# itshawi/data-accelerator

Measured on AMD Instinct MI355X. Metric: events/sec (node) + p99 latency, SimulatedData IoT Flow, higher is better.
Workload: dtype fp64/int64 columns (no reduced precision)

## Files before the change

dxa/ops/csrc/inflate.hip:

```cpp
#include "dxa_common.h"

namespace {

constexpr int IG = 16;
constexpr int WG = 128;
constexpr int LBITS = 9;
constexpr int DBITS = 8;
constexpr int kWaitVm0 = 0xF70;

enum : int32_t { IF_OK = 0, IF_TRUNC = 1, IF_DIST = 2, IF_OVERFLOW = 3, IF_SIZE = 4, IF_CODE = 10, IF_BLOCK = 6 };

struct Tables {
  uint16_t lfast[1 << LBITS];
  uint16_t dfast[1 << DBITS];
  uint16_t lsorted[288];
  uint16_t dsorted[32];
  uint16_t lcount[16];
  uint16_t dcount[16];
  uint8_t lens[320];
  uint8_t clens[20];
  uint16_t csorted[19];
  uint16_t ccount[16];
};

__constant__ uint16_t kLenBase[29] = {3,  4,  5,  6,  7,  8,  9,  10, 11,  13,  15,  17,  19,  23, 27,
                                      31, 35, 43, 51, 59, 67, 83, 99, 115, 131, 163, 195, 227, 258};
__constant__ uint8_t kLenExtra[29] = {0, 0, 0, 0, 0, 0, 0, 0, 1, 1, 1, 1, 2, 2, 2, 2, 3, 3, 3, 3, 4, 4, 4, 4, 5, 5, 5, 5, 0};
__constant__ uint16_t kDistBase[30] = {1,   2,   3,   4,   5,   7,    9,    13,   17,   25,   33,   49,    65,    97,    129,
                                       193, 257, 385, 513, 769, 1025, 1537, 2049, 3073, 4097, 6145, 8193, 12289, 16385, 24577};
__constant__ uint8_t kDistExtra[30] = {0, 0, 0, 0, 1, 1, 2, 2, 3, 3, 4, 4, 5, 5, 6, 6, 7, 7, 8, 8, 9, 9, 10, 10, 11, 11, 12, 12, 13, 13};
__constant__ uint8_t kClenOrder[19] = {16, 17, 18, 0, 8, 7, 9, 6, 10, 5, 11, 4, 12, 3, 13, 2, 14, 1, 15};

__device__ __forceinline__ uint32_t bitrev(uint32_t c, int n) { return __builtin_bitreverse32(c) >> (32 - n); }

__device__ __forceinline__ void lane_sync() {
  __builtin_amdgcn_fence(__ATOMIC_RELEASE, "wavefront");
  __builtin_amdgcn_wave_barrier();
  __builtin_amdgcn_fence(__ATOMIC_ACQUIRE, "wavefront");
}

__device__ bool build_table(const uint8_t* lens, int n, uint16_t* count, uint16_t* sorted, uint16_t* fast, int bits,
                            int maxlen, int gl) {
  lane_sync();
  if (fast) {
    for (int i = gl; i < (1 << bits); i += IG) fast[i] = 0;
    lane_sync();
  }
  uint16_t cnt[16];
  for (int l = 0; l < 16; ++l) cnt[l] = 0;
  for (int s = 0; s < n; ++s) cnt[lens[s]]++;
  int left = 1;
  for (int l = 1; l <= maxlen; ++l) {
    left = (left << 1) - cnt[l];
    if (left < 0) return false;
  }
  uint16_t offs[16];
  offs[1] = 0;
  for (int l = 1; l < 15; ++l) offs[l + 1] = offs[l] + cnt[l];
  if (gl == 0) {
    for (int l = 0; l < 16; ++l) count[l] = cnt[l];
  }
  uint32_t next[16];
  uint32_t code = 0;
  next[0] = 0;
  for (int l = 1; l < 16; ++l) {
    next[l] = code;
    code = (code + cnt[l]) << 1;
  }
  for (int s = 0; s < n; ++s) {
    const int l = lens[s];
    if (!l) continue;
    if (gl == 0) sorted[offs[l]] = (uint16_t)s;
    offs[l]++;
    const uint32_t c = next[l]++;
    if (fast && l <= bits) {
      const uint32_t r = bitrev(c, l);
      const uint16_t e = (uint16_t)((l << 9) | s);
      for (int k = gl; k < (1 << (bits - l)); k += IG) fast[r | ((uint32_t)k << l)] = e;
    }
  }
  lane_sync();
  return true;
}

__global__ __launch_bounds__(WG) void inflate_group_kernel(const uint8_t* __restrict__ src,
                                                           const int64_t* __restrict__ comp_off,
                                                           const int32_t* __restrict__ comp_len,
                                                           const uint8_t* __restrict__ kind,
                                                           const int64_t* __restrict__ out_off,
                                                           const int64_t* __restrict__ cap_arr, int64_t nb,
                                                           uint8_t* __restrict__ dst, int64_t* __restrict__ produced,
                                                           int32_t* __restrict__ status) {
  __shared__ Tables tabs[WG / IG];
  Tables& T = tabs[threadIdx.x / IG];
  const int64_t b = ((int64_t)blockIdx.x * WG + threadIdx.x) / IG;
  const int gl = (int)(threadIdx.x & (IG - 1));
  if (b >= nb || kind[b] != 2) return;
  const uint8_t* in = src + comp_off[b];
  const int32_t n = comp_len[b];
  const int64_t cap64 = cap_arr[b];
  uint8_t* out = dst + out_off[b];
  if (n < 0 || cap64 < 0 || cap64 > INT32_MAX) {
    if (gl == 0) status[b] = IF_OVERFLOW;
    return;
  }
  const int32_t cap = (int32_t)cap64;
  const int32_t lim = n + 8;
  uint64_t bb = 0;
  int bc = 0;
  int32_t ip = 0;
  auto ld32 = [&](int32_t p) -> uint32_t {
    if (p + 4 <= lim) {
      const uintptr_t a = reinterpret_cast<uintptr_t>(in + p);
      const uint32_t* w = reinterpret_cast<const uint32_t*>(a & ~(uintptr_t)3);
      const uint32_t sh = (uint32_t)(a & 3) * 8u;
      const uint32_t lo = w[0];
      if (!sh) return lo;
      return (lo >> sh) | (w[1] << (32u - sh));
    }
    uint32_t v = 0;
    for (int i = 0; i < 4; ++i)
      if (p + i < lim) v |= (uint32_t)in[p + i] << (8 * i);
    return v;
  };
  auto refill = [&]() {
    if (bc <= 32) {
      bb |= (uint64_t)ld32(ip) << bc;
      ip += 4;
      bc += 32;
    }
  };
  auto bits = [&](int k) -> uint32_t {
    refill();
    const uint32_t v = (uint32_t)(bb & ((1ull << k) - 1));
    bb >>= k;
    bc -= k;
    return v;
  };
  auto slow = [&](const uint16_t* count, const uint16_t* sorted, int maxlen) -> int {
    refill();
    int code = 0, first = 0, index = 0;
    for (int l = 1; l <= maxlen; ++l) {
      code |= (int)(bb & 1);
      bb >>= 1;
      bc--;
      const int c = count[l];
      if (code - first < c) return sorted[index + code - first];
      index += c;
      first = (first + c) << 1;
      code <<= 1;
    }
    return -1;
  };
  auto decode = [&](const uint16_t* fast, int fbits, const uint16_t* count, const uint16_t* sorted) -> int {
    refill();
    const uint32_t e = fast[bb & ((1u << fbits) - 1)];
    const int l = (int)(e >> 9);
    if (l) {
      bb >>= l;
      bc -= l;
      return (int)(e & 511);
    }
    return slow(count, sorted, 15);
  };
  int32_t op = 0, rc = IF_OK, done = 0;
  bool last = false;
  while (!last && rc == IF_OK) {
    if ((int64_t)ip * 8 - bc > (int64_t)lim * 8) { rc = IF_TRUNC; break; }
    last = bits(1) != 0;
    const uint32_t type = bits(2);
    if (type == 0) {
      const int drop = bc & 7;
      bb >>= drop;
      bc -= drop;
      const uint32_t len = bits(16), nlen = bits(16);
      if ((len ^ 0xffffu) != nlen) { rc = IF_BLOCK; break; }
      const int32_t pos = ip - bc / 8;
      if (pos + (int32_t)len > n) { rc = IF_TRUNC; break; }
      if (op + (int32_t)len > cap) { rc = IF_OVERFLOW; break; }
      for (int32_t c = gl; c < (int32_t)len; c += IG) out[op + c] = in[pos + c];
      op += (int32_t)len;
      ip = pos + (int32_t)len;
      bb = 0;
      bc = 0;
      continue;
    }
    if (type == 3) { rc = IF_BLOCK; break; }
    int nlit = 288, ndist = 30;
    if (type == 1) {
      for (int s = gl; s < 320; s += IG) T.lens[s] = s < 144 ? 8 : s < 256 ? 9 : s < 280 ? 7 : s < 288 ? 8 : 5;
    } else {
      nlit = (int)bits(5) + 257;
      ndist = (int)bits(5) + 1;
      const int ncl = (int)bits(4) + 4;
      if (nlit > 286 || ndist > 30) { rc = IF_BLOCK; break; }
      uint32_t cl[19];
      for (int i = 0; i < 19; ++i) cl[i] = 0;
      for (int i = 0; i < ncl; ++i) cl[kClenOrder[i]] = bits(3);
      if (gl == 0) {
        for (int i = 0; i < 19; ++i) T.clens[i] = (uint8_t)cl[i];
      }
      if (!build_table(T.clens, 19, T.ccount, T.csorted, nullptr, 0, 7, gl)) { rc = IF_CODE + 0; break; }
      int i = 0;
      while (i < nlit + ndist) {
        const int sym = slow(T.ccount, T.csorted, 7);
        if (sym < 0) { rc = IF_CODE + 1; break; }
        if (sym < 16) {
          if (gl == 0) T.lens[i] = (uint8_t)sym;
          ++i;
          continue;
        }
        int rep, val = 0;
        if (sym == 16) {
          if (i == 0) { rc = IF_CODE + 2; break; }
          lane_sync();
          val = T.lens[i - 1];
          rep = 3 + (int)bits(2);
        } else if (sym == 17) {
          rep = 3 + (int)bits(3);
        } else {
          rep = 11 + (int)bits(7);
        }
        if (i + rep > nlit + ndist) { rc = IF_CODE + 3; break; }
        for (int k = gl; k < rep; k += IG) T.lens[i + k] = (uint8_t)val;
        i += rep;
      }
      if (rc != IF_OK) break;
      lane_sync();
      if (T.lens[256] == 0) { rc = IF_CODE + 4; break; }
    }
    if (!build_table(T.lens, nlit, T.lcount, T.lsorted, T.lfast, LBITS, 15, gl) ||
        !build_table(T.lens + nlit, ndist, T.dcount, T.dsorted, T.dfast, DBITS, 15, gl)) {
      rc = IF_CODE + 5;
      break;
    }
    for (;;) {
      if ((int64_t)ip * 8 - bc > (int64_t)lim * 8) { rc = IF_TRUNC; break; }
      const int sym = decode(T.lfast, LBITS, T.lcount, T.lsorted);
      if (sym < 0) { rc = IF_CODE + 6; break; }
      if (sym < 256) {
        if (op >= cap) { rc = IF_OVERFLOW; break; }
        if (gl == 0) out[op] = (uint8_t)sym;
        ++op;
        continue;
      }
      if (sym == 256) break;
      const int li = sym - 257;
      if (li >= 29) { rc = IF_CODE + 7; break; }
      const int32_t len = kLenBase[li] + (int32_t)bits(kLenExtra[li]);
      const int ds = decode(T.dfast, DBITS, T.dcount, T.dsorted);
      if (ds < 0 || ds >= 30) { rc = IF_CODE + 8; break; }
      const int32_t dist = kDistBase[ds] + (int32_t)bits(kDistExtra[ds]);
      if (dist > op) { rc = IF_DIST; break; }
      if (len > cap - op) { rc = IF_OVERFLOW; break; }
      const int32_t s0 = op - dist;
      if (s0 + (dist < len ? dist : len) > done) {
        __builtin_amdgcn_s_waitcnt(kWaitVm0);
        asm volatile("" ::: "memory");
        done = op;
      }
      if (dist >= len) {
        for (int32_t c = 0; c < len; c += IG)
          if (c + gl < len) out[op + c + gl] = out[s0 + c + gl];
      } else {
        for (int32_t c = 0; c < len; c += IG) {
          const uint32_t k = (uint32_t)(c + gl);
          if ((int32_t)k < len) out[op + (int32_t)k] = out[s0 + (int32_t)(k % (uint32_t)dist)];
        }
      }
      op += len;
    }
  }
  if (rc == IF_OK && op != cap) rc = IF_SIZE;
  if (gl == 0) {
    status[b] = rc;
    produced[b] = op;
  }
}

}

DXA_API int dxa_inflate_into(const void* src, const void* comp_off, const void* comp_len, const void* kind,
                             const void* out_off, const void* cap, int64_t nb, void* dst, void* produced, void* status,
                             void* st) {
  if (nb <= 0) return 0;
  hipLaunchKernelGGL(inflate_group_kernel, dim3((unsigned)((nb * IG + WG - 1) / WG)), dim3(WG), 0, (hipStream_t)st,
                     (const uint8_t*)src, (const int64_t*)comp_off, (const int32_t*)comp_len, (const uint8_t*)kind,
                     (const int64_t*)out_off, (const int64_t*)cap, nb, (uint8_t*)dst, (int64_t*)produced,
                     (int32_t*)status);
  return (int)hipGetLastError();
}
```

Baseline: 251.8 million.

## Stage compressed input via cooperative lane windows and parallelize Huffman table build

Replaces per-lane unaligned 32-bit input loads with a cooperative scheme: each of the 16 lanes in a group loads one word of a 16-word window, and the bit reader pulls words through ds_bpermute, prefetching the next window. Huffman table construction is parallelized with shared atomic histograms and per-length sorted fill, and fast-table entries now pre-encode length and distance base and extra-bit info so the constant-memory lookups go away. Match copies defer their store by one iteration so the load and store overlap. This adds complexity and cross-lane shuffles, and the bit-reader edge cases and delayed-store ordering bring correctness risk.

```diff
diff --git a/dxa/ops/csrc/inflate.hip b/dxa/ops/csrc/inflate.hip
--- a/dxa/ops/csrc/inflate.hip
+++ b/dxa/ops/csrc/inflate.hip
@@ -21,15 +21,39 @@
   uint8_t clens[20];
   uint16_t csorted[19];
   uint16_t ccount[16];
+  uint32_t bcnt[16];
+  uint16_t boffs[16];
+  uint16_t bnext[16];
 };
 
-__constant__ uint16_t kLenBase[29] = {3,  4,  5,  6,  7,  8,  9,  10, 11,  13,  15,  17,  19,  23, 27,
-                                      31, 35, 43, 51, 59, 67, 83, 99, 115, 131, 163, 195, 227, 258};
-__constant__ uint8_t kLenExtra[29] = {0, 0, 0, 0, 0, 0, 0, 0, 1, 1, 1, 1, 2, 2, 2, 2, 3, 3, 3, 3, 4, 4, 4, 4, 5, 5, 5, 5, 0};
-__constant__ uint16_t kDistBase[30] = {1,   2,   3,   4,   5,   7,    9,    13,   17,   25,   33,   49,    65,    97,    129,
-                                       193, 257, 385, 513, 769, 1025, 1537, 2049, 3073, 4097, 6145, 8193, 12289, 16385, 24577};
-__constant__ uint8_t kDistExtra[30] = {0, 0, 0, 0, 1, 1, 2, 2, 3, 3, 4, 4, 5, 5, 6, 6, 7, 7, 8, 8, 9, 9, 10, 10, 11, 11, 12, 12, 13, 13};
-__constant__ uint8_t kClenOrder[19] = {16, 17, 18, 0, 8, 7, 9, 6, 10, 5, 11, 4, 12, 3, 13, 2, 14, 1, 15};
+enum : int { K_PLAIN = 0, K_LITLEN = 1, K_DIST = 2 };
+constexpr uint32_t E_SPECIAL = 0x8000u;
+
+constexpr uint64_t kClenOrderLo = 16ull | 17ull << 5 | 18ull << 10 | 0ull << 15 | 8ull << 20 | 7ull << 25 | 9ull << 30 |
+                                  6ull << 35 | 10ull << 40 | 5ull << 45 | 11ull << 50 | 4ull << 55;
+constexpr uint64_t kClenOrderHi = 12ull | 3ull << 5 | 13ull << 10 | 2ull << 15 | 14ull << 20 | 1ull << 25 | 15ull << 30;
+
+__device__ __forceinline__ int clen_order(int i) {
+  return (int)((i < 12 ? kClenOrderLo >> (5 * i) : kClenOrderHi >> (5 * (i - 12))) & 31);
+}
+
+__device__ __forceinline__ uint32_t lentry(int s) {
+  if (s < 256) return (uint32_t)s << 4;
+  if (s == 256) return E_SPECIAL | (7u << 12);
+  const int li = s - 257;
+  if (li >= 29) return E_SPECIAL | (6u << 12);
+  if (li == 28) return E_SPECIAL | (255u << 4);
+  const int x = li < 4 ? 0 : (li >> 2) - 1;
+  const int base3 = li < 4 ? li : (4 + (li & 3)) << x;
+  return E_SPECIAL | ((uint32_t)x << 12) | ((uint32_t)base3 << 4);
+}
+
+__device__ __forceinline__ uint32_t dentry(int s) {
+  if (s >= 30) return E_SPECIAL;
+  const int x = s < 2 ? 0 : (s >> 1) - 1;
+  const int m = s < 2 ? s : 2 | (s & 1);
+  return ((uint32_t)m << 8) | ((uint32_t)x << 4);
+}
 
 __device__ __forceinline__ uint32_t bitrev(uint32_t c, int n) { return __builtin_bitreverse32(c) >> (32 - n); }
 
@@ -39,44 +63,53 @@
   __builtin_amdgcn_fence(__ATOMIC_ACQUIRE, "wavefront");
 }
 
-__device__ bool build_table(const uint8_t* lens, int n, uint16_t* count, uint16_t* sorted, uint16_t* fast, int bits,
-                            int maxlen, int gl) {
+template <int KIND>
+__device__ bool build_table(Tables& T, const uint8_t* lens, int n, uint16_t* count, uint16_t* sorted, uint16_t* fast,
+                            int bits, int maxlen, int gl) {
+  T.bcnt[gl] = 0;
+  if (fast) {
+    for (int i = gl; i < (1 << bits); i += IG) fast[i] = 0;
+  }
+  lane_sync();
+  for (int s = gl; s < n; s += IG) atomicAdd(&T.bcnt[lens[s] & 15], 1u);
+  lane_sync();
+  int left = 1;
+  bool ok = true;
+  uint32_t off = 0, code = 0, slot = 0;
+  for (int l = 1; l < 16; ++l) {
+    const uint32_t c = T.bcnt[l];
+    if (l <= maxlen) {
+      left = (left << 1) - (int)c;
+      ok = ok && left >= 0;
+    }
+    if (gl == l) {
+      slot = off;
+      T.boffs[l] = (uint16_t)off;
+      T.bnext[l] = (uint16_t)code;
+      count[l] = (uint16_t)c;
+    }
+    off += c;
+    code = (code + c) << 1;
+  }
+  if (!ok) return false;
+  if (gl == 0) {
+    count[0] = (uint16_t)T.bcnt[0];
+  } else {
+#pragma unroll 4
+    for (int s = 0; s < n; ++s) {
+      if (lens[s] == gl) sorted[slot++] = (uint16_t)s;
+    }
+  }
   lane_sync();
   if (fast) {
-    for (int i = gl; i < (1 << bits); i += IG) fast[i] = 0;
-    lane_sync();
-  }
-  uint16_t cnt[16];
-  for (int l = 0; l < 16; ++l) cnt[l] = 0;
-  for (int s = 0; s < n; ++s) cnt[lens[s]]++;
-  int left = 1;
-  for (int l = 1; l <= maxlen; ++l) {
-    left = (left << 1) - cnt[l];
-    if (left < 0) return false;
-  }
-  uint16_t offs[16];
-  offs[1] = 0;
-  for (int l = 1; l < 15; ++l) offs[l + 1] = offs[l] + cnt[l];
-  if (gl == 0) {
-    for (int l = 0; l < 16; ++l) count[l] = cnt[l];
-  }
-  uint32_t next[16];
-  uint32_t code = 0;
-  next[0] = 0;
-  for (int l = 1; l < 16; ++l) {
-    next[l] = code;
-    code = (code + cnt[l]) << 1;
-  }
-  for (int s = 0; s < n; ++s) {
-    const int l = lens[s];
-    if (!l) continue;
-    if (gl == 0) sorted[offs[l]] = (uint16_t)s;
-    offs[l]++;
-    const uint32_t c = next[l]++;
-    if (fast && l <= bits) {
+    for (uint32_t j = gl; j < off; j += IG) {
+      const int s = sorted[j];
+      const int l = lens[s] & 15;
+      if (l > bits) continue;
+      const uint32_t c = (uint32_t)T.bnext[l] + (j - T.boffs[l]);
       const uint32_t r = bitrev(c, l);
-      const uint16_t e = (uint16_t)((l << 9) | s);
-      for (int k = gl; k < (1 << (bits - l)); k += IG) fast[r | ((uint32_t)k << l)] = e;
+      const uint16_t e = (uint16_t)((KIND == K_LITLEN ? lentry(s) : dentry(s)) | (uint32_t)l);
+      for (uint32_t k = 0; k < (1u << (bits - l)); ++k) fast[r | (k << l)] = e;
     }
   }
   lane_sync();
@@ -100,45 +133,68 @@
   const int32_t n = comp_len[b];
   const int64_t cap64 = cap_arr[b];
   uint8_t* out = dst + out_off[b];
-  if (n < 0 || cap64 < 0 || cap64 > INT32_MAX) {
+  if (n < 0 || n > INT32_MAX - 64 || cap64 < 0 || cap64 > INT32_MAX) {
     if (gl == 0) status[b] = IF_OVERFLOW;
     return;
   }
   const int32_t cap = (int32_t)cap64;
   const int32_t lim = n + 8;
+  const int32_t skip = (int32_t)(reinterpret_cast<uintptr_t>(in) & 3);
+  const uint32_t* w = reinterpret_cast<const uint32_t*>(in - skip);
+  const int32_t avail = skip + lim;
+  const int32_t nfull = avail >> 2;
+  uint32_t tail = 0;
+  for (int i = 0; i < (avail & 3); ++i) tail |= (uint32_t)in[nfull * 4 - skip + i] << (8 * i);
+  auto ldw = [&](int32_t k) -> uint32_t { return w[k < nfull ? k : nfull - 1]; };
+  const int lbase = (int)(threadIdx.x & 63 & ~(IG - 1)) << 2;
   uint64_t bb = 0;
   int bc = 0;
-  int32_t ip = 0;
-  auto ld32 = [&](int32_t p) -> uint32_t {
-    if (p + 4 <= lim) {
-      const uintptr_t a = reinterpret_cast<uintptr_t>(in + p);
-      const uint32_t* w = reinterpret_cast<const uint32_t*>(a & ~(uintptr_t)3);
-      const uint32_t sh = (uint32_t)(a & 3) * 8u;
-      const uint32_t lo = w[0];
-      if (!sh) return lo;
-      return (lo >> sh) | (w[1] << (32u - sh));
-    }
-    uint32_t v = 0;
-    for (int i = 0; i < 4; ++i)
-      if (p + i < lim) v |= (uint32_t)in[p + i] << (8 * i);
-    return v;
+  int32_t wn = 0;
+  uint32_t cur = 0, nwin = 0, nxt = 0;
+  auto raw = [&](int32_t k) -> uint32_t {
+    return (uint32_t)__builtin_amdgcn_ds_bpermute(lbase + ((k & (IG - 1)) << 2), (int)cur);
+  };
+  auto pick = [&](uint32_t v, int32_t k) -> uint32_t {
+    return k < nfull ? v : k == nfull ? tail : 0u;
+  };
+  auto fetch = [&]() {
+    if ((wn & (IG - 1)) == 0) {
+      asm volatile("v_mov_b32 %0, %1" : "=v"(cur) : "v"(nwin));
+      nwin = ldw(wn + IG + gl);
+    }
+    nxt = raw(wn);
+  };
+  auto seek = [&](int32_t p) {
+    const int32_t a = skip + p, k = a >> 2, r = (a & 3) * 8;
+    cur = ldw((k & ~(IG - 1)) + gl);
+    nwin = ldw((k & ~(IG - 1)) + IG + gl);
+    bb = pick(raw(k), k) >> r;
+    bc = 32 - r;
+    wn = k + 1;
+    fetch();
   };
   auto refill = [&]() {
     if (bc <= 32) {
-      bb |= (uint64_t)ld32(ip) << bc;
-      ip += 4;
+      bb |= (uint64_t)pick(nxt, wn) << bc;
       bc += 32;
-    }
-  };
-  auto bits = [&](int k) -> uint32_t {
-    refill();
-    const uint32_t v = (uint32_t)(bb & ((1ull << k) - 1));
+      ++wn;
+      fetch();
+    }
+  };
+  auto take = [&](int k) -> uint32_t {
+    const uint32_t v = (uint32_t)bb & ((1u << k) - 1);
     bb >>= k;
     bc -= k;
     return v;
   };
+  auto bits = [&](int k) -> uint32_t {
+    refill();
+    return take(k);
+  };
+  auto past_end = [&]() -> bool {
+    return ((int64_t)wn * 4 - skip) * 8 - bc > (int64_t)lim * 8;
+  };
   auto slow = [&](const uint16_t* count, const uint16_t* sorted, int maxlen) -> int {
-    refill();
     int code = 0, first = 0, index = 0;
     for (int l = 1; l <= maxlen; ++l) {
       code |= (int)(bb & 1);
@@ -152,37 +208,42 @@
     }
     return -1;
   };
-  auto decode = [&](const uint16_t* fast, int fbits, const uint16_t* count, const uint16_t* sorted) -> int {
-    refill();
-    const uint32_t e = fast[bb & ((1u << fbits) - 1)];
-    const int l = (int)(e >> 9);
+  auto decode = [&](const uint16_t* fast, int fbits, const uint16_t* count, const uint16_t* sorted,
+                    bool litlen) -> int {
+    const uint32_t e = fast[(uint32_t)bb & ((1u << fbits) - 1)];
+    const int l = (int)(e & 15);
     if (l) {
       bb >>= l;
       bc -= l;
-      return (int)(e & 511);
-    }
-    return slow(count, sorted, 15);
+      return (int)(e >> 4);
+    }
+    const int s = slow(count, sorted, 15);
+    if (s < 0) return -1;
+    return (int)((litlen ? lentry(s) : dentry(s)) >> 4);
   };
   int32_t op = 0, rc = IF_OK, done = 0;
+  uint32_t mval = 0;
+  int32_t mpos = -1;
+  auto drain = [&]() {
+    if (mpos >= 0) out[mpos] = (uint8_t)mval;
+    mpos = -1;
+  };
+  seek(0);
   bool last = false;
   while (!last && rc == IF_OK) {
-    if ((int64_t)ip * 8 - bc > (int64_t)lim * 8) { rc = IF_TRUNC; break; }
+    if (past_end()) { rc = IF_TRUNC; break; }
     last = bits(1) != 0;
     const uint32_t type = bits(2);
     if (type == 0) {
-      const int drop = bc & 7;
-      bb >>= drop;
-      bc -= drop;
+      take(bc & 7);
       const uint32_t len = bits(16), nlen = bits(16);
       if ((len ^ 0xffffu) != nlen) { rc = IF_BLOCK; break; }
-      const int32_t pos = ip - bc / 8;
+      const int32_t pos = wn * 4 - skip - bc / 8;
       if (pos + (int32_t)len > n) { rc = IF_TRUNC; break; }
       if (op + (int32_t)len > cap) { rc = IF_OVERFLOW; break; }
       for (int32_t c = gl; c < (int32_t)len; c += IG) out[op + c] = in[pos + c];
       op += (int32_t)len;
-      ip = pos + (int32_t)len;
-      bb = 0;
-      bc = 0;
+      seek(pos + (int32_t)len);
       continue;
     }
     if (type == 3) { rc = IF_BLOCK; break; }
@@ -194,15 +255,16 @@
       ndist = (int)bits(5) + 1;
       const int ncl = (int)bits(4) + 4;
       if (nlit > 286 || ndist > 30) { rc = IF_BLOCK; break; }
-      uint32_t cl[19];
-      for (int i = 0; i < 19; ++i) cl[i] = 0;
-      for (int i = 0; i < ncl; ++i) cl[kClenOrder[i]] = bits(3);
-      if (gl == 0) {
-        for (int i = 0; i < 19; ++i) T.clens[i] = (uint8_t)cl[i];
-      }
-      if (!build_table(T.clens, 19, T.ccount, T.csorted, nullptr, 0, 7, gl)) { rc = IF_CODE + 0; break; }
+      for (int s = gl; s < 20; s += IG) T.clens[s] = 0;
+      lane_sync();
+      for (int i = 0; i < ncl; ++i) {
+        const uint32_t v = bits(3);
+        if (gl == 0) T.clens[clen_order(i)] = (uint8_t)v;
+      }
+      if (!build_table<K_PLAIN>(T, T.clens, 19, T.ccount, T.csorted, nullptr, 0, 7, gl)) { rc = IF_CODE + 0; break; }
       int i = 0;
       while (i < nlit + ndist) {
+        refill();
         const int sym = slow(T.ccount, T.csorted, 7);
         if (sym < 0) { rc = IF_CODE + 1; break; }
         if (sym < 16) {
@@ -229,48 +291,52 @@
       lane_sync();
       if (T.lens[256] == 0) { rc = IF_CODE + 4; break; }
     }
-    if (!build_table(T.lens, nlit, T.lcount, T.lsorted, T.lfast, LBITS, 15, gl) ||
-        !build_table(T.lens + nlit, ndist, T.dcount, T.dsorted, T.dfast, DBITS, 15, gl)) {
+    if (!build_table<K_LITLEN>(T, T.lens, nlit, T.lcount, T.lsorted, T.lfast, LBITS, 15, gl) ||
+        !build_table<K_DIST>(T, T.lens + nlit, ndist, T.dcount, T.dsorted, T.dfast, DBITS, 15, gl)) {
       rc = IF_CODE + 5;
       break;
     }
     for (;;) {
-      if ((int64_t)ip * 8 - bc > (int64_t)lim * 8) { rc = IF_TRUNC; break; }
-      const int sym = decode(T.lfast, LBITS, T.lcount, T.lsorted);
-      if (sym < 0) { rc = IF_CODE + 6; break; }
-      if (sym < 256) {
+      if (past_end()) { rc = IF_TRUNC; break; }
+      refill();
+      const int v = decode(T.lfast, LBITS, T.lcount, T.lsorted, true);
+      if (v < 0) { rc = IF_CODE + 6; break; }
+      if (!(v & (int)(E_SPECIAL >> 4))) {
         if (op >= cap) { rc = IF_OVERFLOW; break; }
-        if (gl == 0) out[op] = (uint8_t)sym;
+        if (gl == 0) out[op] = (uint8_t)v;
         ++op;
         continue;
       }
-      if (sym == 256) break;
-      const int li = sym - 257;
-      if (li >= 29) { rc = IF_CODE + 7; break; }
-      const int32_t len = kLenBase[li] + (int32_t)bits(kLenExtra[li]);
-      const int ds = decode(T.dfast, DBITS, T.dcount, T.dsorted);
-      if (ds < 0 || ds >= 30) { rc = IF_CODE + 8; break; }
-      const int32_t dist = kDistBase[ds] + (int32_t)bits(kDistExtra[ds]);
+      const int lx = (v >> 8) & 7;
+      if (lx == 7) break;
+      if (lx == 6) { rc = IF_CODE + 7; break; }
+      const int32_t len = (v & 255) + 3 + (int32_t)take(lx);
+      refill();
+      const int dv = decode(T.dfast, DBITS, T.dcount, T.dsorted, false);
+      if (dv < 0 || (dv & (int)(E_SPECIAL >> 4))) { rc = IF_CODE + 8; break; }
+      const int dx = dv & 15;
+      const int32_t dist = (((dv >> 4) & 3) << dx) + 1 + (int32_t)take(dx);
       if (dist > op) { rc = IF_DIST; break; }
       if (len > cap - op) { rc = IF_OVERFLOW; break; }
       const int32_t s0 = op - dist;
       if (s0 + (dist < len ? dist : len) > done) {
+        drain();
         __builtin_amdgcn_s_waitcnt(kWaitVm0);
         asm volatile("" ::: "memory");
         done = op;
       }
-      if (dist >= len) {
-        for (int32_t c = 0; c < len; c += IG)
-          if (c + gl < len) out[op + c + gl] = out[s0 + c + gl];
-      } else {
-        for (int32_t c = 0; c < len; c += IG) {
-          const uint32_t k = (uint32_t)(c + gl);
-          if ((int32_t)k < len) out[op + (int32_t)k] = out[s0 + (int32_t)(k % (uint32_t)dist)];
+      for (int32_t c = 0; c < len; c += IG) {
+        const int32_t k = c + gl;
+        drain();
+        if (k < len) {
+          mval = out[s0 + (dist >= len ? k : (int32_t)((uint32_t)k % (uint32_t)dist))];
+          mpos = op + k;
         }
       }
       op += len;
     }
   }
+  drain();
   if (rc == IF_OK && op != cap) rc = IF_SIZE;
   if (gl == 0) {
     status[b] = rc;
```

New measurement: 251.7 million. Within noise of the previous version (-0.0%).
